# PeterCalifano/gtsam_PeterCdev

Hardware: AMD Instinct MI355X
Metric: lm_iterations_per_sec (higher is better)
Workload: dtype f64; 1 GPU; bal1723; ordering=schur_nd, replicas=1, parallelism=replicas1

## Files before the change

### gtsam_petercdev_amd/csrc/kernels.h

```cpp
#pragma once
#include <hip/hip_runtime.h>

#include <cstdint>
#include <vector>

namespace gsx {

typedef long long i64;

struct FactorRec {
  i64 jac_off;
  int s0, s1;
  int meas_off, noise_off;
  int type_kind;
  int rows_dim;
};
struct DevProblem {
  int n_vars, n_factors;
  const int *var_type, *var_dim, *var_state_off, *var_tan_off;
  const int *f_type, *f_rows, *f_key_ptr, *f_vars, *f_noise_kind, *f_cols;
  const i64 *f_meas_off, *f_noise_off, *f_jac_off;
  const double *meas, *noise;
  const FactorRec* frec;
  const int* f_active;
  int n_active;
};

struct TermRec {
  i64 jac;
  int m, colA, colB, dB, dst, pad;
};

struct VarRec {
  i64 h_off, hmap_off;
  int dA, rows, loc, toff;
};
struct LeafRec {
  i64 off, h_off, hmap_off, gidx_ptr;
  int n, F, nfv, lean;
  int dA, rows, loc, toff;
  int fvar_ptr, front, pad0, pad1;
};
struct ChildRec {
  i64 src0, cmap_off;
  int nc, s1, pad0, pad1;
};
struct FrontRec {
  i64 off;
  int n, F, nfv, fvar_ptr, child_ptr, nchild;
};

struct DevSymbolic {
  int n_fronts;
  const i64* fr_off;
  const int *fr_N, *fr_F, *fr_nfv, *fr_fvar_ptr, *fvars, *fr_parent, *fr_child_ptr, *children;
  const int* fr_lean;
  const i64 *cmap_ptr, *gidx_ptr;
  const int *cmap, *gidx;
  const i64 *h_off, *hmap_ptr;
  const int *h_rows, *hmap, *h_loc;
  const i64* term_ptr;
  const TermRec* terms;
  const VarRec* var_recs;
  const ChildRec* child_recs;
// ... 83 lines not shown
                         const double* H, const double* damp, const double* scalars, double* arena, DevStatus* status,
                         hipStream_t st);
void launch_front_tree_med(const DevProblem& P, const DevSymbolic& S, const TreeArgs& T, size_t lds_bytes, const double* H,
                           const double* damp, const double* scalars, double* arena, DevStatus* status, hipStream_t st);
void launch_big_init(const DevProblem& P, const DevSymbolic& S, const BigDesc* descs, int count, int max_n,
                     int max_nfv, const double* H, const double* damp, const double* scalars, double* arena,
                     hipStream_t st);
struct BigPlan {
  int chunk = 0;
  std::vector<int> fw, rb, pairs;
  int rounds() const { return (int)fw.size(); }
};
void plan_big_group(const BigDesc* host_descs, int count, BigPlan& plan);
void launch_big_diag(const BigDesc* descs, int count, const BigPlan& plan, int round, double* arena, DevStatus* status,
                     hipStream_t st);
#ifdef GSX_STAMP
void big_stamp_dump(const char* what);
#endif
void launch_big_rows(const BigDesc* descs, int count, const BigPlan& plan, int round, double* arena, hipStream_t st);
void launch_big_schur(const BigDesc* descs, int count, const BigPlan& plan, int round, double* arena, hipStream_t st);
void launch_front_leaf(const DevProblem& P, const DevSymbolic& S, const LeafRec* recs, int count, int max_panel, int threads,
                       const double* H, const double* damp, const double* scalars, double* arena, DevStatus* status,
                       hipStream_t st);
struct GatherSrc {
  i64 off;
  int d2;
  int ldF;
};
struct GatherSeg {
  i64 dst;
  i64 src;
  int n, ld, dims;
  int slot;
};
struct GatherArgs {
  const GatherSeg* segs;
  const GatherSrc* srcs;
  const i64* gt_dst;
  const int *gt_ld, *gt_dims, *gm_task, *gm_slot, *gm_nslots;
  double* scratch;
};
void launch_big_gather(const GatherArgs& G, int seg0, int nseg, int m0, int nm, double* arena, hipStream_t st);
void launch_backsolve(const DevSymbolic& S, const int* ids, int count, int threads, int max_n, const double* arena,
                      double* delta, DevStatus* status, hipStream_t st);
size_t backsolve_big_lds(int max_n, int max_F, int max_sep_rows);
void launch_backsolve_big(const DevSymbolic& S, const int* ids, int count, int max_n, int max_F, const double* arena,
// ... 66 lines not shown
```

### gtsam_petercdev_amd/csrc/kernels.hip

```cpp
#include <hip/hip_runtime.h>

#include <climits>
#include <cstdio>
#include <cstdlib>

#include "device_geometry.h"
#include "gsx_internal.h"
#include "kernels.h"

namespace gsx {
using namespace gsxd;

#define T kTile

__device__ __forceinline__ double wave_sum(double v) {
#pragma unroll
  for (int o = 32; o > 0; o >>= 1) v += __shfl_down(v, o, 64);
  return v;
}
typedef double v4d __attribute__((ext_vector_type(4)));
__device__ __forceinline__ i64 readlane_i64(i64 v, int src_lane) {
  int lo = (int)(v & 0xFFFFFFFFll), hi = (int)(v >> 32);
  lo = __builtin_amdgcn_readlane(lo, src_lane);
  hi = __builtin_amdgcn_readlane(hi, src_lane);
// ... 978 lines not shown
        for (int r0 = 0; r0 < m; r0 += 4) {
          const int r = r0 + lk;
          const double xv = (li <= d && r < m) ? jac[off + (i64)col * m + r] : 0.0;
          acc = __builtin_amdgcn_mfma_f64_16x16x4f64(xv, xv, acc, 0, 0, 0);
        }
        ++q;
      }
    }
  }
#pragma unroll
  for (int qq = 0; qq < 4; ++qq) red[wave][(lk + 4 * qq) * 16 + li] = acc[qq];
  __syncthreads();
  double* out = H + S.h_off[v];
  for (int e = threadIdx.x; e < 256; e += blockDim.x) {
    const int i = e >> 4, j = e & 15;
    if (i <= d && j < d) out[i + j * rows] = ((red[0][e] + red[1][e]) + red[2][e]) + red[3][e];
  }
}
__global__ void __launch_bounds__(256) assemble_h_diag_kernel(DevProblem P, DevSymbolic S, const int* vars, const double* jac,
                                                              double* H) {
  assemble_h_diag_body(P, S, vars, jac, H, blockIdx.x);
}

__global__ void __launch_bounds__(256) assemble_h_star_kernel(DevProblem P, DevSymbolic S, const int* vars, int count,
                                                              const double* jac, double* H) {
  const int lane = threadIdx.x & 63;
  const int w = __builtin_amdgcn_readfirstlane(blockIdx.x * 4 + (threadIdx.x >> 6));
  if (w >= count) return;
  const int v = vars[w];
  const int d = P.var_dim[v], rows = S.h_rows[v];
  const i64 t0 = S.term_ptr[v];
  const int nf = (int)((S.term_ptr[v + 1] - t0) / 3);
  double* panel = H + S.h_off[v];
  const TermRec a0 = S.terms[t0], b0 = S.terms[t0 + 1], c0 = S.terms[t0 + 2];
  const int m = a0.m, colA = a0.colA, colB = b0.colB, dB = b0.dB, colR = c0.colB;
  const int nper = dB * d, nown = d * d + d;
  int ci = 0, cj = 0, odst = 0;
  if (lane < d * d) {
    const int i = lane % d, j = lane / d;
    ci = colA + i; cj = colA + j; odst = i + j * rows;
  } else if (lane < nown) {
    const int j = lane - d * d;
    ci = colR; cj = colA + j; odst = (rows - 1) + j * rows;
  }
  double own = 0.0;
  const float rnper = 1.0f / (float)nper, rdB = 1.0f / (float)dB;
  for (int fb = 0; fb < nf; fb += 64) {
    const int nfb = min(64, nf - fb);
    i64 r_jac = 0;
    int r_dst = 0;
    if (lane < nfb) {
      r_jac = S.terms[t0 + 3 * (i64)(fb + lane)].jac;
      r_dst = S.terms[t0 + 3 * (i64)(fb + lane) + 1].dst;
    }
    const int total = nfb * nper;
    for (int e0 = 0; e0 < total; e0 += 64) {
      const int e = e0 + lane;
      const bool on = e < total;
      int q, rem, i, j;
      divmod_small(on ? e : 0, nper, rnper, q, rem);
      divmod_small(rem, dB, rdB, j, i);
      const int lo = __shfl((int)(r_jac & 0xffffffff), q), hi = __shfl((int)(r_jac >> 32), q);
      const i64 joff = ((i64)hi << 32) | (unsigned)lo;
      const int dst = __shfl(r_dst, q);
      if (on) {
        const double* Jf = jac + joff;
        double acc;
        if (m == 2 && (joff & 1) == 0) {
          const double2 x = reinterpret_cast<const double2*>(Jf)[colB + i];
          const double2 y = reinterpret_cast<const double2*>(Jf)[colA + j];
          acc = x.x * y.x + x.y * y.y;
        } else {
          acc = 0.0;
          for (int r = 0; r < m; ++r) acc += Jf[(colB + i) * m + r] * Jf[(colA + j) * m + r];
        }
        panel[dst + i + j * rows] = acc;
      }
    }
    for (int q = 0; q < nfb; ++q) {
      const i64 joff = readlane_i64(r_jac, q);
      if (lane < nown) {
        const double* Jf = jac + joff;
        if (m == 2 && (joff & 1) == 0) {
          const double2 x = reinterpret_cast<const double2*>(Jf)[ci];
          const double2 y = reinterpret_cast<const double2*>(Jf)[cj];
          own += x.x * y.x + x.y * y.y;
        } else {
          for (int r = 0; r < m; ++r) own += Jf[ci * m + r] * Jf[cj * m + r];
        }
      }
    }
  }
  if (lane < nown) panel[odst] = own;
}

constexpr int kStarVars = 5;
__device__ __forceinline__ void assemble_h_star_bundle_body(const DevProblem& P, const DevSymbolic& S, const int* vars,
                                                            const int2* bundles, int count, const double* jac, double* H,
                                                            int bid) {
  const int lane = threadIdx.x & 63;
  const int w = __builtin_amdgcn_readfirstlane(bid * 4 + (threadIdx.x >> 6));
  if (w >= count) return;
  const int2 bd = bundles[w];
  const int nv = bd.y;
  int s_v = 0, s_rows = 0, s_nf = 0;
  i64 s_t0 = 0, s_hoff = 0;
  if (lane < nv) {
    s_v = vars[bd.x + lane];
    s_rows = S.h_rows[s_v];
    s_t0 = S.term_ptr[s_v];
    s_nf = (int)((S.term_ptr[s_v + 1] - s_t0) / 3);
    s_hoff = S.h_off[s_v];
  }
// ... 17 lines not shown
    if (lane < nft) {
      r_jac = S.terms[t0s + 3 * (i64)fl].jac;
      r_dst = S.terms[t0s + 3 * (i64)fl + 1].dst;
    }
  }
  const i64 t00 = readlane_i64(s_t0, 0);
  const TermRec a0 = S.terms[t00], b0 = S.terms[t00 + 1], c0t = S.terms[t00 + 2];
  const int m = a0.m, colA = a0.colA, colB = b0.colB, dB = b0.dB, colR = c0t.colB;
  const int nper = dB * d, nown = d * d + d;
  const int f_rows = __shfl(s_rows, f_slot);
  const i64 f_hoff = ((i64)__shfl((int)(s_hoff >> 32), f_slot) << 32) | (unsigned)__shfl((int)(s_hoff & 0xffffffff), f_slot);
  const float rnper = 1.0f / (float)nper, rdB = 1.0f / (float)dB;
  const int total = nft * nper;
  for (int e0 = 0; e0 < total; e0 += 64) {
    const int e = e0 + lane;
    const bool on = e < total;
    int q, rem, i, j;
    divmod_small(on ? e : 0, nper, rnper, q, rem);
    divmod_small(rem, dB, rdB, j, i);
    const i64 joff = ((i64)__shfl((int)(r_jac >> 32), q) << 32) | (unsigned)__shfl((int)(r_jac & 0xffffffff), q);
    const int dst = __shfl(r_dst, q);
    const int rows = __shfl(f_rows, q);
    const i64 hoff = ((i64)__shfl((int)(f_hoff >> 32), q) << 32) | (unsigned)__shfl((int)(f_hoff & 0xffffffff), q);
    if (on) {
      const double* Jf = jac + joff;
      double acc;
      if (m == 2 && (joff & 1) == 0) {
        const double2 x = reinterpret_cast<const double2*>(Jf)[colB + i];
        const double2 y = reinterpret_cast<const double2*>(Jf)[colA + j];
        acc = x.x * y.x + x.y * y.y;
      } else {
        acc = 0.0;
        for (int r = 0; r < m; ++r) acc += Jf[(colB + i) * m + r] * Jf[(colA + j) * m + r];
      }
      H[hoff + dst + i + j * rows] = acc;
    }
  }
  {
    int slot, ent;
    divmod_small(lane, nown, 1.0f / (float)nown, slot, ent);
    const bool on = slot < nv;
    const int sl = on ? slot : 0;
    const int rows = __shfl(s_rows, sl), first = __shfl(s_first, sl), nf = __shfl(s_nf, sl);
    const i64 hoff = ((i64)__shfl((int)(s_hoff >> 32), sl) << 32) | (unsigned)__shfl((int)(s_hoff & 0xffffffff), sl);
    int ci, cj, odst;
    if (ent < d * d) {
      const int i = ent % d, j = ent / d;
      ci = colA + i; cj = colA + j; odst = i + j * rows;
    } else {
      const int j = ent - d * d;
      ci = colR; cj = colA + j; odst = (rows - 1) + j * rows;
    }
    int nfmax = 0;
#pragma unroll
    for (int k = 0; k < kStarVars; ++k) nfmax = max(nfmax, k < nv ? __builtin_amdgcn_readlane(s_nf, k) : 0);
    double own = 0.0;
    for (int it = 0; it < nfmax; ++it) {
      const int q = min(first + it, 63);
      const i64 joff = ((i64)__shfl((int)(r_jac >> 32), q) << 32) | (unsigned)__shfl((int)(r_jac & 0xffffffff), q);
      if (on && it < nf) {
        const double* Jf = jac + joff;
        if (m == 2 && (joff & 1) == 0) {
          const double2 x = reinterpret_cast<const double2*>(Jf)[ci];
          const double2 y = reinterpret_cast<const double2*>(Jf)[cj];
          own += x.x * y.x + x.y * y.y;
        } else {
          for (int r = 0; r < m; ++r) own += Jf[ci * m + r] * Jf[cj * m + r];
        }
      }
    }
    if (on) H[hoff + odst] = own;
  }
}
__global__ void __launch_bounds__(256) assemble_h_star_bundle_kernel(DevProblem P, DevSymbolic S, const int* vars,
                                                                    const int2* bundles, int count, const double* jac,
                                                                    double* H) {
  assemble_h_star_bundle_body(P, S, vars, bundles, count, jac, H, blockIdx.x);
}
__global__ void __launch_bounds__(256) assemble_h_diag_star_kernel(DevProblem P, DevSymbolic S, const int* dvars, int dcount,
                                                                  const int* svars, const int2* bundles, int scount,
                                                                  const double* jac, double* H) {
  if ((int)blockIdx.x < dcount) assemble_h_diag_body(P, S, dvars, jac, H, blockIdx.x);
  else assemble_h_star_bundle_body(P, S, svars, bundles, scount, jac, H, (int)blockIdx.x - dcount);
}
void launch_assemble_h_star_bundles(const DevProblem& P, const DevSymbolic& S, const int* vars, const int2* bundles,
                                    int count, const double* jac, double* H, hipStream_t st) {
  if (count) assemble_h_star_bundle_kernel<<<(count + 3) / 4, 256, 0, st>>>(P, S, vars, bundles, count, jac, H);
}
void launch_assemble_h_diag_star(const DevProblem& P, const DevSymbolic& S, const int* dvars, int dcount, const int* svars,
                                 const int2* bundles, int scount, const double* jac, double* H, hipStream_t st) {
  assemble_h_diag_star_kernel<<<dcount + (scount + 3) / 4, 256, 0, st>>>(P, S, dvars, dcount, svars, bundles, scount, jac, H);
}
// ... 1232 lines not shown
  } else {
    bad = !(e1 > -12);
  }
  if (bad) report_failure(status, front[k]);
}
void launch_cond_check(int n, const i64* last, const i64* prev, const int* front, const double* arena, DevStatus* status,
                       hipStream_t st) {
  if (n > 0) cond_check_kernel<<<(n + 255) / 256, 256, 0, st>>>(n, last, prev, front, arena, status);
}

void launch_front_leaf(const DevProblem& P, const DevSymbolic& S, const LeafRec* recs, int count, int max_panel, int threads,
                       const double* H, const double* damp, const double* scalars, double* arena, DevStatus* status,
                       hipStream_t st) {
  if (!count) return;
  static const bool pack_on = std::getenv("GSX_LEAF_PACK") != nullptr;
  if (pack_on && threads == 64 && (size_t)max_panel * sizeof(double) * 4 <= 32 * 1024)
    front_leaf_kernel<true><<<(count + 3) / 4, 256, (size_t)max_panel * sizeof(double) * 4, st>>>(
        P, S, recs, count, max_panel, H, damp, scalars, arena, status);
  else
    front_leaf_kernel<false><<<count, threads, (size_t)max_panel * sizeof(double), st>>>(P, S, recs, count, 0, H, damp,
                                                                                          scalars, arena, status);
}

constexpr int kLG = 4;
struct LeanGroup {
  double x[kLG], y[kLG];
};
template <bool SAME>
__device__ __forceinline__ void lean_group_load(LeanGroup& g, const double* arena, i64 rec_off, int rec_d2, int rec_ldF,
                                                int first, int cnt, int li, int lk, bool rowB, bool colA) {
#pragma unroll
  for (int i = 0; i < kLG; ++i) {
    const int src = first + i;
    const i64 off = readlane_i64(rec_off, src & 63);
    const int ldF = __builtin_amdgcn_readlane(rec_ldF, src & 63);
    const double* pb = arena + off;
    const unsigned o = (unsigned)li + (unsigned)lk * (unsigned)(ldF & 0xFFFFFF);
    const bool in = i < cnt && lk < (ldF >> 24);
    g.x[i] = (rowB && in) ? pb[o] : 0.0;
    if (SAME) {
      g.y[i] = g.x[i];
    } else {
      const int d2 = __builtin_amdgcn_readlane(rec_d2, src & 63);
      g.y[i] = (colA && in) ? pb[(i64)d2 + o] : 0.0;
    }
  }
// ... 459 lines not shown
```

### gtsam_petercdev_amd/csrc/solver.hip

```cpp
#include <hip/hip_runtime.h>

#include <algorithm>
#include <cstdlib>
#include <chrono>
#include <climits>
#include <cmath>
#include <cstdio>
#include <cstring>
#include <limits>
#include <array>
#include <map>
#include <string>
#include <vector>

#include "gsx_internal.h"
#include "kernels.h"

using namespace gsx;

namespace {

#define HIPCHK(ctx, expr)                                                                  \
  do {                                                                                     \
    hipError_t e__ = (expr);                                                               \
// ... 126 lines not shown
    int first = 0, count = 0, max_n = 0;
  };
  std::vector<ConLevel> con_level;
  std::vector<int> con_desc_of_front;
  DevBuf<ConDesc> d_con_descs;
  DevBuf<int> d_con_own_col_ptr, d_con_own_cols, d_con_own_m, d_con_child, d_con_fwd_map, d_con_iwork;
  DevBuf<i64> d_con_own_jac;
  DevBuf<double> d_con_work;
  ConTables CT{};
  int con_hd_n = 0;
  DevBuf<int> d_con_hd_tan, d_con_hd_ptr;
  DevBuf<i64> d_con_hd_jidx;
  DevBuf<double> d_con_hd_w;
  bool constrained() const { return !S.con_fronts.empty(); }
  std::vector<BigDesc> big_descs;
  int big_max_n = 0, big_max_nfv = 0;
  struct HGroup {
    int begin, count, threads, lds;
    bool global;
  };
  std::vector<HGroup> hgroups;
  DevBuf<int2> d_star_bundles;
  int n_star_bundles = 0;
  DevBuf<double> d_values, d_trial, d_delta, d_udelta, d_jac, d_H, d_arena, d_hdiag, d_damp, d_partials, d_scalars;
  DevBuf<double> d_dlu, d_dld;
  DevBuf<DevStatus> d_status;
  double* h_scalars = nullptr;
  DevStatus* h_status = nullptr;
  static constexpr int kPartials = 4096;
  bool values_set = false, linearized = false, h_ready = false, hdiag_ready = false, solved = false, damp_ready = false;
  bool lin0_ready = false;
  bool fact_valid = false;
  double fact_lambda = 0.0;
  bool fact_pending = false;
  int damp_kind = -1;
  double damp_min = 0, damp_max = 0;
  double lm_lambda = 0, lm_factor = 0, lm_error = 0;
  int lm_iterations = 0, lm_inner = 0;
  Timer timers[PH_COUNT];
  int profiling = -1;
  int64_t n_cheirality = 0;
  std::vector<LeafRec> h_leaf_recs;
  std::vector<GatherSeg> h_gsegs;
  std::vector<int> hv_list, hv_group_of_var, hv_pos;
  std::vector<int> fr_sched_pos, fr_group;
  std::vector<int> fr_seg_ptr, fr_segs, seg_level;
// ... 743 lines not shown
      srcs[i] = GatherSrc{(i64)S.off[ch] + S.gs_loc[i], lean ? S.gs_loc2[i] - S.gs_loc[i] : 0,
                          S.N[ch] | (lean ? S.F[ch] << 24 : 0)};
    }
    std::vector<GatherSeg> segs(S.gseg_task.size());
    for (size_t i = 0; i < segs.size(); ++i) {
      const int t = S.gseg_task[i];
      segs[i] = GatherSeg{(i64)S.gt_dst[t], (i64)S.gseg_begin[i], (int)(S.gseg_end[i] - S.gseg_begin[i]), S.gt_ld[t],
                          S.gt_dims[t], S.gseg_slot[i]};
    }
    HIPCHK(c, c->d_gt_dst.upload(std::vector<i64>(S.gt_dst.begin(), S.gt_dst.end()), st));
    HIPCHK(c, c->d_gt_ld.upload(S.gt_ld, st));
    HIPCHK(c, c->d_gt_dims.upload(S.gt_dims, st));
    HIPCHK(c, c->d_gsrcs.upload(srcs, st));
    c->h_gsegs = segs;
    HIPCHK(c, c->d_gsegs.upload(segs, st));
    HIPCHK(c, c->d_gm_task.upload(S.gm_task, st));
    HIPCHK(c, c->d_gm_slot.upload(S.gm_slot, st));
    HIPCHK(c, c->d_gm_nslots.upload(S.gm_nslots, st));
    HIPCHK(c, c->d_gscratch.alloc((size_t)std::max(S.g_max_slots, 1) * 256));
    HIPCHK(c, hipStreamSynchronize(st));
    c->GA = GatherArgs{c->d_gsegs.p, c->d_gsrcs.p, c->d_gt_dst.p, c->d_gt_ld.p, c->d_gt_dims.p, c->d_gm_task.p,
                       c->d_gm_slot.p, c->d_gm_nslots.p, c->d_gscratch.p};
  }
  DevSymbolic& D = c->DS;
  D.n_fronts = S.n_fronts;
  D.fr_off = c->d_fr_off.p; D.fr_N = c->d_fr_N.p; D.fr_F = c->d_fr_F.p; D.fr_nfv = c->d_fr_nfv.p;
  D.fr_fvar_ptr = c->d_fr_fvar_ptr.p; D.fvars = c->d_fvars.p; D.fr_parent = c->d_fr_parent.p;
  D.fr_lean = c->d_fr_lean.p;
  D.fr_child_ptr = c->d_fr_child_ptr.p; D.children = c->d_children.p;
  D.cmap_ptr = c->d_cmap_ptr.p; D.gidx_ptr = c->d_gidx_ptr.p; D.cmap = c->d_cmap.p; D.gidx = c->d_gidx.p;
  D.h_off = c->d_h_off.p; D.hmap_ptr = c->d_hmap_ptr.p; D.h_rows = c->d_h_rows.p; D.hmap = c->d_hmap.p;
  D.h_loc = c->d_h_loc.p;
  D.term_ptr = c->d_term_ptr.p; D.terms = c->d_terms.p;
  D.var_recs = c->d_var_recs.p; D.child_recs = c->d_child_recs.p;
  D.front_recs = c->d_front_recs.p; D.fvar_recs = c->d_fvar_recs.p;
  HIPCHK(c, hipStreamSynchronize(st));
  c->h_ready = false;
  c->solved = false;
  c->fact_valid = c->fact_pending = false;
  c->wf_all_replaced = true;
  c->wf_delta_valid = false;
  c->damp_ready = c->hdiag_ready = false;
  if (c->sharded()) c->linearized = false;
  return GSX_OK;
}

// ... 10 lines not shown
void dev_linearize(gsx_context* c) {
  timer_begin(c, PH_LINEARIZE);
  hipMemsetAsync(&c->d_status.p->n_cheirality, 0, sizeof(int), c->stream);
  const int* lists[6] = {c->d_type_list[0].p, c->d_type_list[1].p, c->d_type_list[2].p, c->d_type_list[3].p,
                         c->d_type_list[4].p, c->d_type_list[5].p};
  launch_linearize(c->DP, lists, c->type_count, c->d_values.p, c->d_jac.p, c->d_status.p, c->stream);
  timer_end(c, PH_LINEARIZE);
  c->sc_dirty |= kXLin;
  c->linearized = true;
  c->lin0_ready = false;
  c->fact_valid = false;
  c->h_ready = false;
  if (c->damp_kind != 0) c->damp_ready = false;
  c->solved = false;
}

void dev_assemble_h(gsx_context* c) {
  timer_begin(c, PH_ASSEMBLE_H);
  const gsx_context::HGroup *gs = nullptr, *gd = nullptr;
  for (const auto& g : c->hgroups) {
    if (g.threads == -1 && c->n_star_bundles) gs = &g;
    if (g.threads == 0 && g.count > 0) gd = &g;
  }
  const bool fused = gs && gd;
  if (fused)
    launch_assemble_h_diag_star(c->DP, c->DS, c->d_hvars.p + gd->begin, gd->count, c->d_hvars.p + gs->begin,
                                c->d_star_bundles.p, c->n_star_bundles, c->d_jac.p, c->d_H.p, c->stream);
  for (const auto& g : c->hgroups) {
    if (fused && (&g == gs || &g == gd)) continue;
    if (g.threads == -1 && c->n_star_bundles) {
      launch_assemble_h_star_bundles(c->DP, c->DS, c->d_hvars.p + g.begin, c->d_star_bundles.p, c->n_star_bundles,
                                     c->d_jac.p, c->d_H.p, c->stream);
      continue;
    }
    launch_assemble_h_group(c->DP, c->DS, c->d_hvars.p + g.begin, g.count, g.threads, g.lds, g.global, c->d_jac.p,
                            c->d_H.p, c->stream);
  }
  timer_end(c, PH_ASSEMBLE_H);
  c->h_ready = true;
  c->hdiag_ready = false;
}

void dev_hessian_diag(gsx_context* c) {
  if (c->hdiag_ready) return;
  launch_hessian_diag(c->DP, c->DS, c->d_H.p, c->d_hdiag.p, c->stream);
  if (c->con_hd_n)
    launch_constraint_hdiag(c->con_hd_n, c->d_con_hd_tan.p, c->d_con_hd_ptr.p, c->d_con_hd_jidx.p, c->d_con_hd_w.p,
                            c->d_jac.p, c->d_hdiag.p, c->stream);
  if (c->sharded()) {
    launch_mask_copy(c->d_hdiag.p, c->d_sched_tan.p, c->P.tan_size, c->d_hdiag.p, c->stream);
    shard_allreduce(c, c->d_hdiag.p, c->P.tan_size);
  }
  c->hdiag_ready = true;
}

void dev_damping(gsx_context* c, int diagonal, double mind, double maxd) {
  if (c->damp_ready && c->damp_kind == diagonal && (diagonal == 0 || (c->damp_min == mind && c->damp_max == maxd))) return;
  if (diagonal) dev_hessian_diag(c);
  launch_make_damping((int)c->P.tan_size, c->d_hdiag.p, diagonal, mind, maxd, c->d_damp.p, c->stream);
  if (c->sharded()) launch_mask_copy(c->d_damp.p, c->d_own_tan.p, c->P.tan_size, c->d_damp.p, c->stream);
  c->damp_ready = true;
  c->damp_kind = diagonal;
  c->damp_min = mind;
  c->damp_max = maxd;
}

void dev_big_factor(gsx_context* c, const BigDesc* descs, int count, const BigPlan& plan, hipStream_t st, bool prof) {
  for (int r = 0; r < plan.rounds(); ++r) {
    if (prof) timer_begin(c, PH_K_POTRF0);
    launch_big_diag(descs, count, plan, r, c->d_arena.p, c->d_status.p, st);
    if (prof) timer_end(c, PH_K_POTRF0);
    if (prof) timer_begin(c, PH_K_TRSM);
    launch_big_rows(descs, count, plan, r, c->d_arena.p, st);
    if (prof) timer_end(c, PH_K_TRSM);
    if (prof) timer_begin(c, PH_K_SYRK);
    launch_big_schur(descs, count, plan, r, c->d_arena.p, st);
    if (prof) timer_end(c, PH_K_SYRK);
  }
}

void debug_sync(gsx_context* c, const char* what, int a, int b) {
  static const bool on = std::getenv("GSX_DEBUG_LAUNCH") != nullptr;
  if (!on) return;
  fprintf(stderr, "[gsx] %s (%d, %d) ...", what, a, b);
  fflush(stderr);
  const hipError_t e = hipStreamSynchronize(c->stream);
  const hipError_t e2 = hipGetLastError();
  fprintf(stderr, " %s / %s\n", hipGetErrorString(e), hipGetErrorString(e2));
  fflush(stderr);
}

bool bulk_ready(gsx_context* c) {
  if (c->bulk) return true;
  int least = 0, greatest = 0;
  if (hipDeviceGetStreamPriorityRange(&least, &greatest) != hipSuccess) return false;
  if (hipStreamCreateWithPriority(&c->bulk, hipStreamNonBlocking, least) != hipSuccess) {
    c->bulk = nullptr;
    return false;
  }
  if (hipEventCreateWithFlags(&c->bulk_go, hipEventDisableTiming) != hipSuccess ||
      hipEventCreateWithFlags(&c->bulk_done, hipEventDisableTiming) != hipSuccess)
    return false;
  return true;
}

void dev_factorize(gsx_context* c, double lambda) {
  const Symbolic& S = c->S;
  c->fact_valid = false;
  c->fact_pending = true;
  c->fact_lambda = lambda;
  c->wf_all_replaced = true;
  c->sc_dirty |= kXFact;
  timer_begin(c, PH_FACTORIZE);
  launch_begin_factorization(c->d_scalars.p, lambda, c->d_status.p, c->d_tree_cursor.p, c->stream);
  if (!c->big_descs.empty())
    launch_big_init(c->DP, c->DS, c->d_big.p, (int)c->big_descs.size(), c->big_max_n, c->big_max_nfv, c->d_H.p,
                    c->d_damp.p, c->d_scalars.p, c->d_arena.p, c->stream);
  const int sg = S.n_ulevels;
  const bool have_side = S.side_level0 >= 0;
  const bool use_bulk = have_side && c->profiling <= 0 && bulk_ready(c);
  if (S.n_levels > 0) {
    const std::vector<SmallLaunch>& LL = c->leaf_launch[0];
    const size_t n_main_leaf = c->leaf_side_group0 != (size_t)-1 ? c->leaf_side_group0 : LL.size();
    if (use_bulk) {
      hipEventRecord(c->bulk_go, c->stream);
      hipStreamWaitEvent(c->bulk, c->bulk_go, 0);
      for (size_t g = n_main_leaf; g < LL.size(); ++g) {
        const SmallLaunch& sl = LL[g];
        launch_front_leaf(c->DP, c->DS, c->d_leaf_recs.p + (sl.begin - c->leaf_base), sl.count, sl.max_panel, sl.threads,
                          c->d_H.p, c->d_damp.p, c->d_scalars.p, c->d_arena.p, c->d_status.p, c->bulk);
      }
      launch_big_gather(c->GA, S.gseg_lvl_ptr[sg], S.gseg_lvl_ptr[sg + 1] - S.gseg_lvl_ptr[sg], S.gm_lvl_ptr[sg],
                        S.gm_lvl_ptr[sg + 1] - S.gm_lvl_ptr[sg], c->d_arena.p, c->bulk);
      hipEventRecord(c->bulk_done, c->bulk);
      c->bulk_pending = true;
    }
    for (size_t g = 0; g < (use_bulk ? n_main_leaf : LL.size()); ++g) {
      const SmallLaunch& sl = LL[g];
      if (c->profiling > 0) timer_begin(c, PH_FACTOR_LEAF);
      launch_front_leaf(c->DP, c->DS, c->d_leaf_recs.p + (sl.begin - c->leaf_base), sl.count, sl.max_panel, sl.threads, c->d_H.p,
                        c->d_damp.p, c->d_scalars.p, c->d_arena.p, c->d_status.p, c->stream);
      if (c->profiling > 0) timer_end(c, PH_FACTOR_LEAF);
    }
  }
  for (size_t t = 0; t < c->tree_tiers.size(); ++t) {
    const gsx_context::TreeTier& tt = c->tree_tiers[t];
    if (!tt.nstart) continue;
    if (c->profiling > 0) timer_begin(c, PH_FACTOR_SMALL);
    const TreeArgs ta{c->d_tree_start.p + tt.start0, tt.nstart, c->d_tree_cursor.p + t, c->d_tree_pending.p,
                      c->d_tree_up.p, c->d_tree_npend.p};
    if (tt.med_lds)
      launch_front_tree_med(c->DP, c->DS, ta, tt.med_lds, c->d_H.p, c->d_damp.p, c->d_scalars.p, c->d_arena.p,
                            c->d_status.p, c->stream);
    else
      launch_front_tree(c->DP, c->DS, ta, tt.max_n, tt.threads, c->d_H.p, c->d_damp.p, c->d_scalars.p, c->d_arena.p,
                        c->d_status.p, c->stream);
    debug_sync(c, tt.med_lds ? "front_tree_med" : "front_tree", tt.nstart, (int)tt.med_lds);
    if (c->profiling > 0) timer_end(c, PH_FACTOR_SMALL);
  }
  for (int l = 0; l < S.n_ulevels; ++l) {
    for (const SmallLaunch& sl : c->rest_launch[l]) {
      if (c->profiling > 0) timer_begin(c, PH_FACTOR_SMALL);
      launch_lds_group(c->DP, c->DS, c->d_rest_ids.p + sl.begin, sl, c->d_H.p, c->d_damp.p, c->d_scalars.p, c->d_arena.p,
                       c->d_status.p, c->stream);
// ... 327 lines not shown
}

extern "C" {

const char* gsx_version(void) { return "gsx 0.1.0 (gfx950)"; }

int32_t gsx_device_count(void) {
  int n = 0;
  if (hipGetDeviceCount(&n) != hipSuccess) return 0;
  return n;
}

gsx_status gsx_create(const gsx_problem_desc* desc, int32_t device, gsx_handle* out) {
  if (!out) return GSX_E_INVALID;
  *out = nullptr;
  gsx_context* c = new gsx_context();
  gsx_status st = lower_problem(desc, c->P, c->err);
  if (st != GSX_OK) {
    std::fprintf(stderr, "gsx_create: %s\n", c->err.c_str());
    delete c;
    return st;
  }
  c->device = device;
  int n = 0;
  if (hipGetDeviceCount(&n) == hipSuccess && n > 0 && device >= 0 && device < n && hipSetDevice(device) == hipSuccess &&
      hipStreamCreate(&c->stream) == hipSuccess) {
    c->has_device = true;
    st = upload_problem(c);
    if (st != GSX_OK) {
      std::fprintf(stderr, "gsx_create: %s\n", c->err.c_str());
      delete c;
      return st;
    }
  }
  *out = c;
  return GSX_OK;
}

gsx_status gsx_destroy(gsx_handle h) {
  if (!h) return GSX_OK;
  if (h->has_device) {
    hipSetDevice(h->device);
    hipStreamSynchronize(h->stream);
    for (auto& t : h->timers) {
      for (auto& ev : t.pending) t.pool.push_back(ev);
      for (auto& ev : t.pool) {
// ... 591 lines not shown
    HIPCHK(h, h->d_dlu.alloc(std::max<int64_t>(nt, 1)));
    HIPCHK(h, h->d_dld.alloc(std::max<int64_t>(nt, 1)));
  }
  st = compute_error_sync(h, &h->lm_error);
  if (st != GSX_OK) return st;
  h->lm_iterations = 0;
  double delta = delta_initial;
  Trace tr{r};
  if (r) {
    r->initial_error = h->lm_error;
    r->trace_len = 0;
    r->n_solve_failures = 0;
  }
  double currentError = h->lm_error;
  if (!(currentError <= errTol) && max_iterations > 0) {
    double newError = currentError;
    do {
      currentError = newError;
      dev_linearize(h);
      dev_assemble_h(h);
      dev_damping(h, 0, 0, 0);
      dev_factorize(h, 0.0);
      dev_backsolve(h);
      launch_gradient(h->DP, h->DS, h->d_H.p, h->d_dlu.p, h->stream);
      launch_vec_dot(h->d_dlu.p, h->d_dlu.p, nt, h->d_partials.p, gsx_context::kPartials, h->d_scalars.p, SC_DOT0, h->stream);
      launch_ax_sqnorm(h->DP, h->d_jac.p, h->d_dlu.p, h->d_partials.p, gsx_context::kPartials, h->d_scalars.p, SC_DOT1,
                       h->stream);
      launch_vec_dot(h->d_delta.p, h->d_delta.p, nt, h->d_partials.p, gsx_context::kPartials, h->d_scalars.p, SC_DOT2,
                     h->stream);
      launch_vec_dot(h->d_dlu.p, h->d_delta.p, nt, h->d_partials.p, gsx_context::kPartials, h->d_scalars.p, SC_DOT3,
                     h->stream);
      st = readback(h);
      if (st != GSX_OK) return st;
      if (h->h_status->n_fail > 0 || h->h_status->n_nonfinite > 0) {
        h->err = "indeterminate linear system";
        return GSX_E_INDETERMINATE;
      }
      const double gg = h->h_scalars[SC_DOT0], ag2 = h->h_scalars[SC_DOT1];
      const double step = gg / ag2;
      const double uu = step * step * gg, nn = h->h_scalars[SC_DOT2], un = step * h->h_scalars[SC_DOT3];
      const double f_error = h->lm_error;
      double result_f = f_error, cu = 0, cn = 0;
      bool stay = true, zero_step = false;
      while (stay) {
        dogleg_coefficients(delta, uu, nn, un, &cu, &cn);
        launch_vec_axpby(h->d_dld.p, cu * step, h->d_dlu.p, cn, h->d_delta.p, nt, h->stream);
// ... 61 lines not shown
      else if (t == GSX_F_PROJECTION) lists[4].push_back(f);
      else if (t == GSX_F_BEARINGRANGE) lists[5].push_back(f);
      else if (t == GSX_F_BETWEEN && vt == GSX_VAR_POSE2) lists[1].push_back(f);
      else if (t == GSX_F_BETWEEN && vt == GSX_VAR_POSE3) lists[2].push_back(f);
      else if (t != GSX_F_LINEAR) lists[3].push_back(f);
    }
    const int* lp[6];
    int cnt[6];
    for (int k = 0; k < 6; ++k) {
      HIPCHK(h, ps.lists[k].stage(lists[k], sm));
      lp[k] = ps.lists[k].p;
      cnt[k] = (int)lists[k].size();
    }
    timer_begin(h, PH_LINEARIZE);
    launch_linearize(h->DP, lp, cnt, h->d_values.p, h->d_jac.p, h->d_status.p, sm);
    timer_end(h, PH_LINEARIZE);
  }
  h->lin0_ready = false;
  return GSX_OK;
}
gsx_status partial_assemble(gsx_handle h, std::vector<int>& dvar) {
  hipStream_t sm = h->stream;
  gsx_context::PartialScratch& ps = h->ps;
  {
    std::sort(dvar.begin(), dvar.end(), [&](int a, int b) { return h->hv_pos[a] < h->hv_pos[b]; });
    std::vector<std::pair<int, int>> ranges(h->hgroups.size(), {0, 0});
    for (size_t i = 0; i < dvar.size(); ++i) {
      std::pair<int, int>& r = ranges[h->hv_group_of_var[dvar[i]]];
      if (!r.second) r.first = (int)i;
      r.second++;
    }
    HIPCHK(h, ps.hv.stage(dvar, sm));
    timer_begin(h, PH_ASSEMBLE_H);
    for (size_t g = 0; g < h->hgroups.size(); ++g)
      if (ranges[g].second)
        launch_assemble_h_group(h->DP, h->DS, ps.hv.p + ranges[g].first, ranges[g].second, h->hgroups[g].threads,
                                h->hgroups[g].lds, h->hgroups[g].global, h->d_jac.p, h->d_H.p, sm);
    timer_end(h, PH_ASSEMBLE_H);
    h->hdiag_ready = false;
  }
  return GSX_OK;
}
gsx_status partial_factor(gsx_handle h, std::vector<int>& dfr) {
  if (!h->wf_all_replaced) {
    HIPCHK(h, h->wf_flags_ready(h->stream));
    HIPCHK(h, h->d_wf_ids.stage(dfr, h->stream));
// ... 874 lines not shown
```

Baseline: 558.7 LM iterations/s.

## Fuse star-variable Hessian assembly into leaf front factorization kernel

Adds a front_star_leaf kernel that, for lean single-variable leaf fronts of star-group variables (small point blocks fed by 2-row factors), builds the point block, its damping and Cholesky, and the eliminated off-diagonal rows straight from the Jacobian. This skips assembling those Hessian panels before factorization. The full star-panel assembly is deferred to dev_ensure_hstar, which runs only when the Hessian diagonal, gradient or partial assembly actually needs it. The aim is to cut Hessian-panel traffic on the factorization path and to avoid reassembly across damping retries. The cost is an extra deferred assembly each iteration, plus more setup code and extra paths to keep in sync. The inline star dot-product code is also factored into helpers.

```diff
diff --git a/gtsam_petercdev_amd/csrc/kernels.h b/gtsam_petercdev_amd/csrc/kernels.h
--- a/gtsam_petercdev_amd/csrc/kernels.h
+++ b/gtsam_petercdev_amd/csrc/kernels.h
@@ -40,6 +40,14 @@
   int n, F, nfv, lean;
   int dA, rows, loc, toff;
   int fvar_ptr, front, pad0, pad1;
+};
+constexpr int kStarMaxD = 3;
+struct StarLeafRec {
+  i64 off, h_off, t0;
+  i64 jac0, prow_off;
+  int n, nf, d, toff;
+  int colA, colB, colR, dB;
+  int front, jstride, rrow, pad0;
 };
 struct ChildRec {
   i64 src0, cmap_off;
@@ -169,6 +177,9 @@
 void launch_front_leaf(const DevProblem& P, const DevSymbolic& S, const LeafRec* recs, int count, int max_panel, int threads,
                        const double* H, const double* damp, const double* scalars, double* arena, DevStatus* status,
                        hipStream_t st);
+void launch_front_star_leaf(const DevSymbolic& S, const StarLeafRec* recs, int count, const int* prow, const double* jac,
+                            const double* damp, const double* scalars, double* H, double* arena, DevStatus* status,
+                            hipStream_t st);
 struct GatherSrc {
   i64 off;
   int d2;
diff --git a/gtsam_petercdev_amd/csrc/kernels.hip b/gtsam_petercdev_amd/csrc/kernels.hip
--- a/gtsam_petercdev_amd/csrc/kernels.hip
+++ b/gtsam_petercdev_amd/csrc/kernels.hip
@@ -1024,6 +1024,21 @@
   assemble_h_diag_body(P, S, vars, jac, H, blockIdx.x);
 }
 
+__device__ __forceinline__ double star_pair_dot(double2 x, double2 y) { return x.x * y.x + x.y * y.y; }
+__device__ __forceinline__ double star_entry(const double* Jf, int m, bool pair, int ci, int cj) {
+  if (pair) return star_pair_dot(reinterpret_cast<const double2*>(Jf)[ci], reinterpret_cast<const double2*>(Jf)[cj]);
+  double acc = 0.0;
+  for (int r = 0; r < m; ++r) acc += Jf[ci * m + r] * Jf[cj * m + r];
+  return acc;
+}
+__device__ __forceinline__ void star_accum(double& own, const double* Jf, int m, bool pair, int ci, int cj) {
+  if (pair) {
+    own += star_pair_dot(reinterpret_cast<const double2*>(Jf)[ci], reinterpret_cast<const double2*>(Jf)[cj]);
+  } else {
+    for (int r = 0; r < m; ++r) own += Jf[ci * m + r] * Jf[cj * m + r];
+  }
+}
+
 __global__ void __launch_bounds__(256) assemble_h_star_kernel(DevProblem P, DevSymbolic S, const int* vars, int count,
                                                               const double* jac, double* H) {
   const int lane = threadIdx.x & 63;
@@ -1065,32 +1080,11 @@
       const int lo = __shfl((int)(r_jac & 0xffffffff), q), hi = __shfl((int)(r_jac >> 32), q);
       const i64 joff = ((i64)hi << 32) | (unsigned)lo;
       const int dst = __shfl(r_dst, q);
-      if (on) {
-        const double* Jf = jac + joff;
-        double acc;
-        if (m == 2 && (joff & 1) == 0) {
-          const double2 x = reinterpret_cast<const double2*>(Jf)[colB + i];
-          const double2 y = reinterpret_cast<const double2*>(Jf)[colA + j];
-          acc = x.x * y.x + x.y * y.y;
-        } else {
-          acc = 0.0;
-          for (int r = 0; r < m; ++r) acc += Jf[(colB + i) * m + r] * Jf[(colA + j) * m + r];
-        }
-        panel[dst + i + j * rows] = acc;
-      }
+      if (on) panel[dst + i + j * rows] = star_entry(jac + joff, m, m == 2 && (joff & 1) == 0, colB + i, colA + j);
     }
     for (int q = 0; q < nfb; ++q) {
       const i64 joff = readlane_i64(r_jac, q);
-      if (lane < nown) {
-        const double* Jf = jac + joff;
-        if (m == 2 && (joff & 1) == 0) {
-          const double2 x = reinterpret_cast<const double2*>(Jf)[ci];
-          const double2 y = reinterpret_cast<const double2*>(Jf)[cj];
-          own += x.x * y.x + x.y * y.y;
-        } else {
-          for (int r = 0; r < m; ++r) own += Jf[ci * m + r] * Jf[cj * m + r];
-        }
-      }
+      if (lane < nown) star_accum(own, jac + joff, m, m == 2 && (joff & 1) == 0, ci, cj);
     }
   }
   if (lane < nown) panel[odst] = own;
@@ -1154,19 +1148,7 @@
     const int dst = __shfl(r_dst, q);
     const int rows = __shfl(f_rows, q);
     const i64 hoff = ((i64)__shfl((int)(f_hoff >> 32), q) << 32) | (unsigned)__shfl((int)(f_hoff & 0xffffffff), q);
-    if (on) {
-      const double* Jf = jac + joff;
-      double acc;
-      if (m == 2 && (joff & 1) == 0) {
-        const double2 x = reinterpret_cast<const double2*>(Jf)[colB + i];
-        const double2 y = reinterpret_cast<const double2*>(Jf)[colA + j];
-        acc = x.x * y.x + x.y * y.y;
-      } else {
-        acc = 0.0;
-        for (int r = 0; r < m; ++r) acc += Jf[(colB + i) * m + r] * Jf[(colA + j) * m + r];
-      }
-      H[hoff + dst + i + j * rows] = acc;
-    }
+    if (on) H[hoff + dst + i + j * rows] = star_entry(jac + joff, m, m == 2 && (joff & 1) == 0, colB + i, colA + j);
   }
   {
     int slot, ent;
@@ -1190,16 +1172,7 @@
     for (int it = 0; it < nfmax; ++it) {
       const int q = min(first + it, 63);
       const i64 joff = ((i64)__shfl((int)(r_jac >> 32), q) << 32) | (unsigned)__shfl((int)(r_jac & 0xffffffff), q);
-      if (on && it < nf) {
-        const double* Jf = jac + joff;
-        if (m == 2 && (joff & 1) == 0) {
-          const double2 x = reinterpret_cast<const double2*>(Jf)[ci];
-          const double2 y = reinterpret_cast<const double2*>(Jf)[cj];
-          own += x.x * y.x + x.y * y.y;
-        } else {
-          for (int r = 0; r < m; ++r) own += Jf[ci * m + r] * Jf[cj * m + r];
-        }
-      }
+      if (on && it < nf) star_accum(own, jac + joff, m, m == 2 && (joff & 1) == 0, ci, cj);
     }
     if (on) H[hoff + odst] = own;
   }
@@ -2478,6 +2451,171 @@
                                                                                           scalars, arena, status);
 }
 
+__device__ __forceinline__ double readlane_f64(double v, int src_lane) {
+  return __longlong_as_double(readlane_i64(__double_as_longlong(v), src_lane));
+}
+__device__ __forceinline__ void as_stored(double& v) { asm volatile("" : "+v"(v)); }
+__global__ void __launch_bounds__(256) front_star_leaf_kernel(DevSymbolic S, const StarLeafRec* recs, int count,
+                                                              const int* prow, const double* jac, const double* damp,
+                                                              const double* scalars, double* H, double* arena,
+                                                              DevStatus* status) {
+  constexpr int D = kStarMaxD;
+  const int lane = threadIdx.x & 63;
+  const int w = __builtin_amdgcn_readfirstlane(blockIdx.x * 4 + (threadIdx.x >> 6));
+  if (w >= count) return;
+  const StarLeafRec rec = recs[w];
+  const int n = rec.n, nf = rec.nf, d = rec.d, dB = rec.dB;
+  const int colA = rec.colA, colB = rec.colB, colR = rec.colR;
+  const TermRec* T = S.terms + rec.t0;
+  const int* pr = prow + rec.prow_off;
+  auto factor_jac = [&](int q) {
+    return jac + (rec.jstride > 0 ? rec.jac0 + (i64)q * rec.jstride : T[3 * (i64)q].jac);
+  };
+  const int npart = nf * dB;
+  const float rdB = 1.0f / (float)dB;
+  auto load_factor = [&](int q, double2* fa, double2& fr) {
+    const double2* J = reinterpret_cast<const double2*>(factor_jac(min(q, nf - 1)));
+#pragma unroll
+    for (int j = 0; j < D; ++j) fa[j] = J[colA + min(j, d - 1)];
+    fr = J[colR];
+  };
+  auto load_row = [&](int p, int& R, double2& xb, double2* ya) {
+    int q, i;
+    p = min(p, npart - 1);
+    divmod_small(p, dB, rdB, q, i);
+    R = pr[p];
+    const double2* J = reinterpret_cast<const double2*>(factor_jac(q));
+    xb = J[colB + i];
+#pragma unroll
+    for (int j = 0; j < D; ++j) ya[j] = J[colA + min(j, d - 1)];
+  };
+  double2 fa[D], fr, xb, ya[D];
+  int R = 0;
+  load_factor(lane, fa, fr);
+  load_row(lane, R, xb, ya);
+  const double lambda = scalars[SC_LAMBDA];
+  double O[D][D], G[D];
+#pragma unroll
+  for (int r = 0; r < D; ++r) {
+    G[r] = 0.0;
+#pragma unroll
+    for (int c = 0; c < D; ++c) O[r][c] = 0.0;
+  }
+  for (int fb = 0; fb < nf; fb += 64) {
+    if (fb > 0) load_factor(fb + lane, fa, fr);
+    const int nfb = min(64, nf - fb);
+    double po[D][D], pg[D];
+#pragma unroll
+    for (int r = 0; r < D; ++r) {
+      pg[r] = star_pair_dot(fr, fa[r]);
+#pragma unroll
+      for (int c = 0; c <= r; ++c) po[r][c] = star_pair_dot(fa[r], fa[c]);
+    }
+    for (int q = 0; q < nfb; ++q) {
+#pragma unroll
+      for (int r = 0; r < D; ++r) {
+        if (r >= d) break;
+        G[r] += readlane_f64(pg[r], q);
+#pragma unroll
+        for (int c = 0; c <= r; ++c) O[r][c] += readlane_f64(po[r][c], q);
+      }
+    }
+  }
+  double L[D][D], inv[D];
+  int fail = 0;
+#pragma unroll
+  for (int r = 0; r < D; ++r) {
+#pragma unroll
+    for (int c = 0; c <= r; ++c) {
+      double x = O[r][c];
+      as_stored(x);
+      if (r == c && r < d) x += lambda * damp[rec.toff + r];
+      as_stored(x);
+      L[r][c] = x;
+    }
+  }
+#pragma unroll
+  for (int j = 0; j < D; ++j) {
+    if (j >= d) break;
+    const double p = L[j][j];
+    if (!(p > 0)) fail = 1;
+    const double s = (p > 0) ? sqrt(p) : 1.0;
+    inv[j] = 1.0 / s;
+#pragma unroll
+    for (int r = j + 1; r < D; ++r) {
+      L[r][j] = L[r][j] * inv[j];
+      as_stored(L[r][j]);
+    }
+    L[j][j] = s;
+#pragma unroll
+    for (int c = j + 1; c < D; ++c) {
+      const double lc = L[c][j];
+#pragma unroll
+      for (int r = c; r < D; ++r) {
+        L[r][c] -= L[r][j] * lc;
+        as_stored(L[r][c]);
+      }
+    }
+  }
+  auto eliminate = [&](double* x) {
+#pragma unroll
+    for (int j = 0; j < D; ++j) {
+      if (j >= d) break;
+      x[j] = x[j] * inv[j];
+      as_stored(x[j]);
+#pragma unroll
+      for (int c = j + 1; c < D; ++c) {
+        x[c] -= x[j] * L[c][j];
+        as_stored(x[c]);
+      }
+    }
+  };
+  double* A = arena + rec.off;
+  for (int p0 = 0; p0 < npart; p0 += 64) {
+    if (p0 > 0) load_row(p0 + lane, R, xb, ya);
+    double x[D];
+#pragma unroll
+    for (int j = 0; j < D; ++j) {
+      x[j] = star_pair_dot(xb, ya[j]);
+      as_stored(x[j]);
+    }
+    eliminate(x);
+    if (p0 + lane < npart) {
+#pragma unroll
+      for (int c = 0; c < D; ++c)
+        if (c < d) A[R + (i64)c * n] = x[c];
+    }
+  }
+  if (lane < d) {
+#pragma unroll
+    for (int r = 0; r < D; ++r)
+      if (lane == r) {
+#pragma unroll
+        for (int c = 0; c <= r; ++c) A[r + (i64)c * n] = L[r][c];
+      }
+  } else if (lane == d) {
+    double x[D];
+#pragma unroll
+    for (int j = 0; j < D; ++j) {
+      x[j] = G[j];
+      as_stored(x[j]);
+      if (j < d) H[rec.h_off + (n - 1) + (i64)j * n] = G[j];
+    }
+    eliminate(x);
+    const int Rg = rec.rrow;
+#pragma unroll
+    for (int c = 0; c < D; ++c)
+      if (c < d) A[Rg + (i64)c * n] = x[c];
+  }
+  if (fail && lane == 0) report_failure(status, rec.front);
+}
+void launch_front_star_leaf(const DevSymbolic& S, const StarLeafRec* recs, int count, const int* prow, const double* jac,
+                            const double* damp, const double* scalars, double* H, double* arena, DevStatus* status,
+                            hipStream_t st) {
+  if (count)
+    front_star_leaf_kernel<<<(count + 3) / 4, 256, 0, st>>>(S, recs, count, prow, jac, damp, scalars, H, arena, status);
+}
+
 constexpr int kLG = 4;
 struct LeanGroup {
   double x[kLG], y[kLG];
diff --git a/gtsam_petercdev_amd/csrc/solver.hip b/gtsam_petercdev_amd/csrc/solver.hip
--- a/gtsam_petercdev_amd/csrc/solver.hip
+++ b/gtsam_petercdev_amd/csrc/solver.hip
@@ -172,6 +172,19 @@
   std::vector<HGroup> hgroups;
   DevBuf<int2> d_star_bundles;
   int n_star_bundles = 0;
+  bool fused_star_env = true;
+  bool fused_star = false;
+  bool hstar_ready = true;
+  struct LeafSplit {
+    int sbegin, scount;
+    int rbegin, rcount;
+  };
+  std::vector<LeafSplit> leaf_split;
+  DevBuf<StarLeafRec> d_star_recs;
+  DevBuf<int> d_star_prow;
+  DevBuf<LeafRec> d_leaf_rest_recs;
+  DevBuf<int> d_star_rest_vars;
+  int n_star_rest = 0;
   DevBuf<double> d_values, d_trial, d_delta, d_udelta, d_jac, d_H, d_arena, d_hdiag, d_damp, d_partials, d_scalars;
   DevBuf<double> d_dlu, d_dld;
   DevBuf<DevStatus> d_status;
@@ -961,6 +974,79 @@
     c->GA = GatherArgs{c->d_gsegs.p, c->d_gsrcs.p, c->d_gt_dst.p, c->d_gt_ld.p, c->d_gt_dims.p, c->d_gm_task.p,
                        c->d_gm_slot.p, c->d_gm_nslots.p, c->d_gscratch.p};
   }
+  c->fused_star = false;
+  c->leaf_split.clear();
+  c->n_star_rest = 0;
+  {
+    int sgrp = -1;
+    for (size_t g = 0; g < c->hgroups.size(); ++g)
+      if (c->hgroups[g].threads == -1) sgrp = (int)g;
+    if (c->fused_star_env && sgrp >= 0 && !c->sharded() && !c->constrained() && S.n_levels > 0) {
+      auto star_leaf = [&](const LeafRec& r) {
+        const int v = S.fvars[S.fvar_ptr[r.front]];
+        if (c->hv_group_of_var[v] != sgrp || r.nfv != 1 || !r.lean || r.F != r.dA || r.dA > kStarMaxD || r.loc != 0 ||
+            r.n != r.rows)
+          return false;
+        const int64_t tb = S.term_ptr[v], te = S.term_ptr[v + 1];
+        const int64_t nf = (te - tb) / 3;
+        if (nf < 1 || nf >= 1024 || r.dA + nf * S.t_dB[tb + 1] + 1 != r.n) return false;
+        for (int64_t t = tb; t < te; t += 3)
+          if (S.t_m[t] != 2 || (S.t_jac[t] & 1)) return false;
+        std::vector<char> seen(r.n, 0);
+        for (int k = 0; k < r.n; ++k) {
+          const int R = S.hmap[S.hmap_ptr[v] + k];
+          if (R < 0 || R >= r.n || seen[R] || (k < r.dA && R != k)) return false;
+          seen[R] = 1;
+        }
+        return true;
+      };
+      std::vector<char> fused_var(P.n_vars, 0);
+      std::vector<StarLeafRec> srec;
+      std::vector<int> prow;
+      std::vector<LeafRec> rrec;
+      for (const SmallLaunch& sl : c->leaf_launch[0]) {
+        gsx_context::LeafSplit ls{(int)srec.size(), 0, (int)rrec.size(), 0};
+        for (int k = sl.begin; k < sl.begin + sl.count; ++k) {
+          const LeafRec& r = c->h_leaf_recs[k - c->leaf_base];
+          if (!star_leaf(r)) {
+            rrec.push_back(r);
+            continue;
+          }
+          const int v = S.fvars[S.fvar_ptr[r.front]];
+          const int64_t tb = S.term_ptr[v];
+          const int nf = (int)((S.term_ptr[v + 1] - tb) / 3), dB = S.t_dB[tb + 1];
+          fused_var[v] = 1;
+          const int64_t stride = nf > 1 ? S.t_jac[tb + 3] - S.t_jac[tb] : 2;
+          bool even = stride > 0 && stride <= (1 << 30);
+          for (int q = 0; q < nf && even; ++q) even = S.t_jac[tb + 3 * q] == S.t_jac[tb] + q * stride;
+          const int* hm = S.hmap.data() + S.hmap_ptr[v];
+          const i64 prow_off = (i64)prow.size();
+          for (int q = 0; q < nf; ++q)
+            for (int i = 0; i < dB; ++i) prow.push_back(hm[S.t_dst[tb + 3 * q + 1] + i]);
+          srec.push_back(StarLeafRec{r.off, r.h_off, (i64)tb, (i64)S.t_jac[tb], prow_off, r.n, nf, r.dA, r.toff,
+                                     S.t_colA[tb], S.t_colB[tb + 1], S.t_colB[tb + 2], dB, r.front, even ? (int)stride : 0,
+                                     hm[r.n - 1], 0});
+        }
+        ls.scount = (int)srec.size() - ls.sbegin;
+        ls.rcount = (int)rrec.size() - ls.rbegin;
+        c->leaf_split.push_back(ls);
+      }
+      if (!srec.empty()) {
+        std::vector<int> rest;
+        const gsx_context::HGroup& g = c->hgroups[sgrp];
+        for (int k = g.begin; k < g.begin + g.count; ++k)
+          if (!fused_var[c->hv_list[k]]) rest.push_back(c->hv_list[k]);
+        c->fused_star = true;
+        c->n_star_rest = (int)rest.size();
+        HIPCHK(c, c->d_star_recs.upload(srec, st));
+        HIPCHK(c, c->d_star_prow.upload(prow, st));
+        if (!rrec.empty()) HIPCHK(c, c->d_leaf_rest_recs.upload(rrec, st));
+        if (!rest.empty()) HIPCHK(c, c->d_star_rest_vars.upload(rest, st));
+      } else {
+        c->leaf_split.clear();
+      }
+    }
+  }
   DevSymbolic& D = c->DS;
   D.n_fronts = S.n_fronts;
   D.fr_off = c->d_fr_off.p; D.fr_N = c->d_fr_N.p; D.fr_F = c->d_fr_F.p; D.fr_nfv = c->d_fr_nfv.p;
@@ -1017,12 +1103,19 @@
     if (g.threads == -1 && c->n_star_bundles) gs = &g;
     if (g.threads == 0 && g.count > 0) gd = &g;
   }
-  const bool fused = gs && gd;
+  const bool fs = c->fused_star;
+  const bool fused = gs && gd && !fs;
   if (fused)
     launch_assemble_h_diag_star(c->DP, c->DS, c->d_hvars.p + gd->begin, gd->count, c->d_hvars.p + gs->begin,
                                 c->d_star_bundles.p, c->n_star_bundles, c->d_jac.p, c->d_H.p, c->stream);
   for (const auto& g : c->hgroups) {
     if (fused && (&g == gs || &g == gd)) continue;
+    if (fs && g.threads == -1) {
+      if (c->n_star_rest)
+        launch_assemble_h_group(c->DP, c->DS, c->d_star_rest_vars.p, c->n_star_rest, -1, 0, false, c->d_jac.p, c->d_H.p,
+                                c->stream);
+      continue;
+    }
     if (g.threads == -1 && c->n_star_bundles) {
       launch_assemble_h_star_bundles(c->DP, c->DS, c->d_hvars.p + g.begin, c->d_star_bundles.p, c->n_star_bundles,
                                      c->d_jac.p, c->d_H.p, c->stream);
@@ -1033,11 +1126,27 @@
   }
   timer_end(c, PH_ASSEMBLE_H);
   c->h_ready = true;
+  c->hstar_ready = !fs;
   c->hdiag_ready = false;
+}
+
+void dev_ensure_hstar(gsx_context* c) {
+  if (c->hstar_ready) return;
+  for (const auto& g : c->hgroups) {
+    if (g.threads != -1) continue;
+    if (c->n_star_bundles)
+      launch_assemble_h_star_bundles(c->DP, c->DS, c->d_hvars.p + g.begin, c->d_star_bundles.p, c->n_star_bundles,
+                                     c->d_jac.p, c->d_H.p, c->stream);
+    else
+      launch_assemble_h_group(c->DP, c->DS, c->d_hvars.p + g.begin, g.count, g.threads, g.lds, g.global, c->d_jac.p,
+                              c->d_H.p, c->stream);
+  }
+  c->hstar_ready = true;
 }
 
 void dev_hessian_diag(gsx_context* c) {
   if (c->hdiag_ready) return;
+  dev_ensure_hstar(c);
   launch_hessian_diag(c->DP, c->DS, c->d_H.p, c->d_hdiag.p, c->stream);
   if (c->con_hd_n)
     launch_constraint_hdiag(c->con_hd_n, c->d_con_hd_tan.p, c->d_con_hd_ptr.p, c->d_con_hd_jidx.p, c->d_con_hd_w.p,
@@ -1083,6 +1192,21 @@
   const hipError_t e2 = hipGetLastError();
   fprintf(stderr, " %s / %s\n", hipGetErrorString(e), hipGetErrorString(e2));
   fflush(stderr);
+}
+
+void dev_leaf_group(gsx_context* c, size_t g, hipStream_t st) {
+  const SmallLaunch& sl = c->leaf_launch[0][g];
+  if (c->fused_star && c->leaf_split[g].scount) {
+    const gsx_context::LeafSplit& ls = c->leaf_split[g];
+    launch_front_star_leaf(c->DS, c->d_star_recs.p + ls.sbegin, ls.scount, c->d_star_prow.p, c->d_jac.p, c->d_damp.p,
+                           c->d_scalars.p, c->d_H.p, c->d_arena.p, c->d_status.p, st);
+    if (ls.rcount)
+      launch_front_leaf(c->DP, c->DS, c->d_leaf_rest_recs.p + ls.rbegin, ls.rcount, sl.max_panel, sl.threads, c->d_H.p,
+                        c->d_damp.p, c->d_scalars.p, c->d_arena.p, c->d_status.p, st);
+    return;
+  }
+  launch_front_leaf(c->DP, c->DS, c->d_leaf_recs.p + (sl.begin - c->leaf_base), sl.count, sl.max_panel, sl.threads, c->d_H.p,
+                    c->d_damp.p, c->d_scalars.p, c->d_arena.p, c->d_status.p, st);
 }
 
 bool bulk_ready(gsx_context* c) {
@@ -1120,21 +1244,15 @@
     if (use_bulk) {
       hipEventRecord(c->bulk_go, c->stream);
       hipStreamWaitEvent(c->bulk, c->bulk_go, 0);
-      for (size_t g = n_main_leaf; g < LL.size(); ++g) {
-        const SmallLaunch& sl = LL[g];
-        launch_front_leaf(c->DP, c->DS, c->d_leaf_recs.p + (sl.begin - c->leaf_base), sl.count, sl.max_panel, sl.threads,
-                          c->d_H.p, c->d_damp.p, c->d_scalars.p, c->d_arena.p, c->d_status.p, c->bulk);
-      }
+      for (size_t g = n_main_leaf; g < LL.size(); ++g) dev_leaf_group(c, g, c->bulk);
       launch_big_gather(c->GA, S.gseg_lvl_ptr[sg], S.gseg_lvl_ptr[sg + 1] - S.gseg_lvl_ptr[sg], S.gm_lvl_ptr[sg],
                         S.gm_lvl_ptr[sg + 1] - S.gm_lvl_ptr[sg], c->d_arena.p, c->bulk);
       hipEventRecord(c->bulk_done, c->bulk);
       c->bulk_pending = true;
     }
     for (size_t g = 0; g < (use_bulk ? n_main_leaf : LL.size()); ++g) {
-      const SmallLaunch& sl = LL[g];
       if (c->profiling > 0) timer_begin(c, PH_FACTOR_LEAF);
-      launch_front_leaf(c->DP, c->DS, c->d_leaf_recs.p + (sl.begin - c->leaf_base), sl.count, sl.max_panel, sl.threads, c->d_H.p,
-                        c->d_damp.p, c->d_scalars.p, c->d_arena.p, c->d_status.p, c->stream);
+      dev_leaf_group(c, g, c->stream);
       if (c->profiling > 0) timer_end(c, PH_FACTOR_LEAF);
     }
   }
@@ -1508,6 +1626,10 @@
     return st;
   }
   c->device = device;
+  {
+    const char* e = std::getenv("GSX_FUSED_STAR");
+    c->fused_star_env = !(e && std::atoi(e) == 0);
+  }
   int n = 0;
   if (hipGetDeviceCount(&n) == hipSuccess && n > 0 && device >= 0 && device < n && hipSetDevice(device) == hipSuccess &&
       hipStreamCreate(&c->stream) == hipSuccess) {
@@ -2145,6 +2267,7 @@
       dev_damping(h, 0, 0, 0);
       dev_factorize(h, 0.0);
       dev_backsolve(h);
+      dev_ensure_hstar(h);
       launch_gradient(h->DP, h->DS, h->d_H.p, h->d_dlu.p, h->stream);
       launch_vec_dot(h->d_dlu.p, h->d_dlu.p, nt, h->d_partials.p, gsx_context::kPartials, h->d_scalars.p, SC_DOT0, h->stream);
       launch_ax_sqnorm(h->DP, h->d_jac.p, h->d_dlu.p, h->d_partials.p, gsx_context::kPartials, h->d_scalars.p, SC_DOT1,
@@ -2252,6 +2375,7 @@
 gsx_status partial_assemble(gsx_handle h, std::vector<int>& dvar) {
   hipStream_t sm = h->stream;
   gsx_context::PartialScratch& ps = h->ps;
+  dev_ensure_hstar(h);
   {
     std::sort(dvar.begin(), dvar.end(), [&](int a, int b) { return h->hv_pos[a] < h->hv_pos[b]; });
     std::vector<std::pair<int, int>> ranges(h->hgroups.size(), {0, 0});
```

Measured after the change: 582.6 LM iterations/s, median of 6. 4.3% higher.
